# zhengjingsen/LidarDetection

Hardware: AMD Instinct MI355X
Metric: frames/sec (fwd+NMS) PointPillar-KITTI (higher is better)
Workload: dtype f32; 1 GPU; PointPillar-KITTI bs=16 per GPU, fp32, eval BN folded: HIP voxelize + PFN; dense 2D backbone = first layer from the pillars (sparse implicit GEMM), stride-1 3x3 layers as Winograd F(4x4,3x3) on the fp32 MFMA, strided deblocks as one fused MFMA GEMM (all this repo's HIP), the two stride-2 3x3 layers MIOpen, stride-1 deblock + 1x1 heads hipBLASLt; exact HIP top-k + decode + batched rotated NMS; clou; replicas=1

## Files before the change

### include/lidar_hip.h

```cpp
#ifndef LIDAR_HIP_H
#define LIDAR_HIP_H

#include <stddef.h>
#include <stdint.h>

#ifdef __cplusplus
extern "C" {
#endif

#define LIDAR_OK 0
#define LIDAR_ERR_ARG (-1)
#define LIDAR_ERR_LAUNCH (-2)
#define LIDAR_ERR_WORKSPACE (-3)
#define LIDAR_ERR_UNSUPPORTED (-4)

size_t lidar_voxelize_workspace_bytes(int batch, int n_max, int max_voxels);
int lidar_voxelize_workspace_init(void *ws, size_t ws_bytes, int batch, int n_max, int max_voxels, void *stream);
int lidar_voxelize(const float *points, const int *point_offsets, int batch, int n_max, int num_features,
                   const float *range6, const float *voxel_size3, const int *grid3, int max_points,
                   int max_voxels, int compact, int algo, float *voxels, int *coords, int *num_points,
                   int *voxel_offsets, void *ws, size_t ws_bytes, void *stream);
int lidar_voxelize_hostoff(const float *points, const int *point_offsets, const int *host_offsets, int batch, int n_max,
                           int num_features, const float *range6, const float *voxel_size3, const int *grid3, int max_points,
                           int max_voxels, int compact, int algo, float *voxels, int *coords, int *num_points,
// ... 136 lines not shown
size_t lidar_spconv_conv_table_workspace_bytes(int n, int kD, int kH, int kW, int sD, int sH, int sW);
int lidar_spconv_conv_outputs(const int *indices, int n, int batch, int D, int H, int W, int kD, int kH, int kW, int sD,
                              int sH, int sW, int pD, int pH, int pW, int *out_indices, int out_cap, int *num_out,
                              void *ws, size_t ws_bytes, void *stream);
int lidar_spconv_conv_tables(int n, int kD, int kH, int kW, int sD, int sH, int sW, int num_out, int *nbr, int *nbr_t,
                             void *ws, size_t ws_bytes, void *stream);
int lidar_spconv_grid_init(int *grid, size_t cells, void *stream);
int lidar_spconv_grid_rows(const int *indices, int n, const int *n_dev, int batch, int D, int H, int W, int *grid, int mode, void *stream);
int lidar_spconv_grid_table(const int *out_indices, int n_out, int batch, int D, int H, int W, int kD, int kH, int kW, int sD, int sH, int sW,
                            int pD, int pH, int pW, const int *grid_in, int limit, int *nbr, void *stream);
int lidar_spconv_grid_table_t(const int *indices, int n, int batch, int D, int H, int W, int kD, int kH, int kW, int sD, int sH, int sW, int pD,
                              int pH, int pW, const int *grid_out, int limit, int *nbr_t, void *stream);
int lidar_spconv_grid_pad_rows(int *out_indices, const int *num_dev, int cap, void *stream);
int lidar_spconv_transpose_table(const int *nbr, int n_out, int K, int n_in, int *nbr_t, void *stream);
size_t lidar_spconv_grid_outputs_workspace_bytes(int n, int K);
int lidar_spconv_grid_outputs(const int *indices, int n, int batch, int D, int H, int W, int kD, int kH, int kW, int sD, int sH, int sW, int pD,
                              int pH, int pW, int *grid_out, int *out_indices, int *num_out, void *ws, size_t ws_bytes,
                              void *stream);
int lidar_spconv_implicit_gemm(const float *in_features, const int *nbr, int n_out, int K, int Cin, int Cout,
                               const float *weight, const float *bias, float *out_features, void *stream);
int lidar_spconv_implicit_gemm_fused(const float *in_features, const int *nbr, int n_out, int K, int Cin, int Cout,
                                     const float *weight, const float *bias, const float *residual, int relu,
                                     float *out_features, void *stream);
int lidar_spconv_row_masks(const int *nbr, int n_out, int K, int *masks, void *stream);
size_t lidar_spconv_mask_group_workspace_bytes(int n_out);
int lidar_spconv_mask_group_init(void *ws, size_t ws_bytes, void *stream);
int lidar_spconv_mask_group(const int *nbr, int n_out, int K, int *masks, int *order, void *ws, size_t ws_bytes, void *stream);
int lidar_spconv_sorted_gemm_supported(int K, int Cin, int Cout);
int lidar_spconv_implicit_gemm_sorted(const float *in_features, const int *nbr, const int *row_mask, const int *order,
                                      int n_out, int K, int Cin, int Cout, const float *weight, const float *bias,
                                      const float *residual, int relu, float *out_features, void *stream);
size_t lidar_spconv_packed_floats(int K, int Cin, int Cout);
int lidar_spconv_pack_weights(const float *weight, int K, int Cin, int Cout, float *packed, void *stream);
int lidar_spconv_implicit_gemm_sorted_packed(const float *in_features, const int *nbr, const int *row_mask, const int *order,
                                             int n_out, int K, int Cin, int Cout, const float *packed, const float *bias,
                                             const float *residual, int relu, float *out_features, void *stream);
int lidar_spconv_wgrad(const float *in_features, const float *grad_out, const int *nbr, int n_out, int K, int Cin, int Cout,
                       float *grad_weight, void *stream);
int lidar_spconv_wgrad_mfma_supported(int K, int Cin, int Cout);
size_t lidar_spconv_wgrad_workspace_bytes(int n_out, int K, int Cin, int Cout);
int lidar_spconv_wgrad_mfma(const float *in_features, const float *grad_out, const int *nbr, const int *order, int n_out, int K,
                            int Cin, int Cout, float *grad_weight, void *ws, size_t ws_bytes, void *stream);
size_t lidar_sparse_to_dense_workspace_bytes(int batch, int D, int H, int W);
int lidar_sparse_to_dense(const float *features, const int *indices, int n, int channels, int batch, int D, int H, int W,
                          float *out, void *ws, size_t ws_bytes, void *stream);

int lidar_bias_act_nhwc(const float *in, const float *bias, long long n_pix, int C, int relu, float *out, int out_C,
                        int out_off, void *stream);
int lidar_bias_act_upsample_nhwc(const float *in, const float *bias, int batch, int h, int w, int s, int C, int relu,
                                 float *out, int out_C, int out_off, void *stream);
int lidar_dense_gemm_bias_act(const float *A, long long M, int K, const float *W, int N, const float *bias, int relu,
                              float *D, int ldd, void *ws, size_t ws_bytes, void *stream);
int lidar_dense_gemm_export_choices(int *out7, int cap);
int lidar_dense_gemm_import_choices(const int *in7, int n);

size_t lidar_wino_packed_floats(int Cin, int Cout);
int lidar_wino_supported(int Cin, int Cout);
int lidar_wino_pack_weights(const float *w, int Cin, int Cout, float *packed, void *stream);
int lidar_wino_conv3x3_nhwc(const float *in, int B, int H, int W, int Cin, const float *packed, const float *bias, int relu, int Cout,
                            float *out, int out_C, int out_off, void *stream);
int lidar_wino_conv3x3_grouped_nhwc(const float *in, int B, int H, int W, int in_C, int group_cin, int n_groups, const float *packed,
                                    const float *bias, int relu, float *out, int out_C, int out_off, void *stream);
int lidar_wino_conv3x3_grouped_compact_nhwc(const float *in, int B, int H, int W, int in_C, int group_cin, int n_groups,
                                            const float *packed, const float *bias, int relu, const int *grp_cout, const int *grp_ooff,
                                            float *out, int out_C, int out_off, void *stream);

size_t lidar_wino43_packed_floats(int Cin, int Cout);
int lidar_wino43_supported(int Cin, int Cout);
int lidar_wino43_pack_weights(const float *w, int Cin, int Cout, float *packed, void *stream);
int lidar_wino43_conv3x3_nhwc(const float *in, int B, int H, int W, int Cin, int in_C, const float *packed, const float *bias, int relu,
                              int Cout, float *out, int out_C, int out_off, void *stream);

int lidar_wino43_wgrad_supported(int Cin, int Cout);
size_t lidar_wino43_wgrad_workspace_bytes(int B, int H, int W, int Cin, int Cout);
int lidar_wino43_wgrad_nhwc(const float *x, int x_ld, const float *g, int g_ld, int B, int H, int W, int Cin, int Cout, float *dw,
                            void *ws, size_t ws_bytes, void *stream);

size_t lidar_deconv_packed_floats(int K, int N);
int lidar_deconv_supported(int K, int s, int C_up);
int lidar_deconv_pack_weights(const float *W, int K, int N, float *packed, void *stream);
int lidar_deconv_gemm_nhwc(const float *in, int B, int h, int w, int K, const float *packed, const float *bias, int relu, int s, int C_up,
                           float *out, int out_C, int out_off, void *stream);

int lidar_anchor_scores(const float *head, long long n_loc, int row_stride, int cls_off, int anchors_per_loc, int num_class,
                        float score_thresh, float *scores, unsigned char *labels, void *stream);
int lidar_decode_topk(const float *head, int batch, long long locs_per_frame, int row_stride, int box_off, int dir_off,
                      int anchors_per_loc, int num_dir_bins, const long long *top_idx, int k, const float *anchors,
                      float dir_offset, float dir_limit_offset, float period, float *boxes, void *stream);
size_t lidar_topk_workspace_bytes(int batch, long long n);
int lidar_topk_workspace_init(void *ws, size_t ws_bytes, int batch, long long n, void *stream);
int lidar_anchor_scores_hist(const float *head, int batch, long long locs_per_frame, int row_stride, int cls_off, int anchors_per_loc,
                             int num_class, float score_thresh, float *scores, unsigned char *labels, void *ws, size_t ws_bytes,
                             void *stream);
int lidar_topk_desc(const float *scores, int batch, long long n, int k, float valid_min, float score_max, int hist_ready,
                    float *top_scores, long long *top_idx, int *counts, void *ws, size_t ws_bytes, void *stream);
int lidar_post_nms_gather(const float *boxes, const float *top_scores, const long long *top_idx, const unsigned char *labels,
                          const long long *keep, const int *num_keep, int batch, int k, long long n, int keep_stride, int post,
                          float *out_boxes, float *out_scores, long long *out_labels, int *out_num, void *stream);

size_t lidar_anchor_assign_workspace_bytes(int batch, int max_gt, int num_classes);
int lidar_anchor_assign(const float *const *anchors, const long long *counts, const long long *per_loc, const long long *out_off,
                        const float *matched, const float *unmatched, const int *remap, int num_classes, int anchor_dim,
                        long long a_total, const signed char *class_of_id, const float *gt, const float *gt_enlarged, int batch,
                        int max_gt, int gt_cols, int code_size, int sincos, int norm_by_num_examples, int *labels, float *targets,
                        float *weights, void *ws, size_t ws_bytes, void *stream);

size_t lidar_anchor_loss_workspace_bytes(int batch, const long long *counts, int num_heads);
int lidar_anchor_loss_forward(const float *const *cls, const float *const *box, const float *const *dir, const long long *counts,
                              const int *cols, const int *col_off, int num_heads, const int *labels, const float *targets,
                              const float *anchors, int anchor_dim, int batch, long long n_total, int num_class, int code_size,
                              int num_dir_bins, const float *code_weights, const float *weights, int flags, float *losses, void *ws,
                              size_t ws_bytes, void *stream);
int lidar_anchor_loss_backward(const float *const *cls, const float *const *box, const float *const *dir, const long long *counts,
                               const int *cols, const int *col_off, int num_heads, const int *labels, const float *targets,
                               const float *anchors, int anchor_dim, int batch, long long n_total, int num_class, int code_size,
                               int num_dir_bins, const float *code_weights, const float *weights, int flags,
                               const float *grad_losses, float *const *d_cls, float *const *d_box, float *const *d_dir, void *ws,
                               size_t ws_bytes, void *stream);

int lidar_sparse_to_bev_nhwc(const float *features, const int *indices, int n, int channels, int batch, int D, int H, int W,
                             float *out, void *ws, size_t ws_bytes, void *stream);

int lidar_rotate_iou_eval(const float *boxes, int n, const float *query_boxes, int k, int criterion, float *iou, void *stream);

int lidar_boxes_iou_bev_cpu(const float *boxes_a, int n_a, const float *boxes_b, int n_b, float *out);
int lidar_points_in_boxes_cpu(const float *boxes, int n_boxes, const float *pts, int n_pts, int *out);

#ifdef __cplusplus
}
#endif
#endif
```

### lidardetection_amd/_lib.py

```python
import ctypes as C
import os

_HERE = os.path.dirname(os.path.abspath(__file__))
SO_PATH = os.environ.get("LIDAR_HIP_SO") or os.path.join(_HERE, "csrc", "liblidar_hip.so")

vp, i32, f32, sz = C.c_void_p, C.c_int, C.c_float, C.c_size_t

SIGNATURES = {
    "lidar_voxelize_workspace_bytes": (sz, [i32, i32, i32]),
    "lidar_voxelize_workspace_init": (i32, [vp, sz, i32, i32, i32, vp]),
    "lidar_voxelize": (i32, [vp, vp, i32, i32, i32, vp, vp, vp, i32, i32, i32, i32, vp, vp, vp, vp, vp, sz, vp]),
    "lidar_voxelize_hostoff": (i32, [vp, vp, vp, i32, i32, i32, vp, vp, vp, i32, i32, i32, i32, vp, vp, vp, vp, vp, sz, vp]),
    "lidar_voxelize_error_flag": (i32, [vp, sz, i32, i32, i32]),
    "lidar_timer_create": (vp, []),
    "lidar_timer_destroy": (None, [vp]),
    "lidar_voxelize_time_next": (None, [vp]),
    "lidar_timer_elapsed_ms": (C.c_float, [vp]),
    "lidar_timer_parts_ms": (i32, [vp, vp]),
    "lidar_voxelize_set_error_mirror": (i32, [vp, sz, i32, i32, i32, vp, vp]),
    "lidar_pillar_vfe": (i32, [vp, vp, vp, i32, vp, i32, i32, vp, vp, vp, i32, vp, vp, i32, i32, i32, vp, vp]),
    "lidar_mean_vfe": (i32, [vp, vp, i32, i32, i32, i32, vp, vp]),
    "lidar_pillar_scatter_workspace_bytes": (sz, [i32, i32, i32]),
    "lidar_pillar_scatter": (i32, [vp, vp, i32, i32, vp, i32, i32, i32, i32, i32, vp, vp, sz, vp]),
    "lidar_pillar_scatter_update": (i32, [vp, vp, i32, i32, vp, i32, i32, i32, i32, vp, vp, vp, vp]),
# ... 14 lines not shown
    "lidar_nms_batch": (i32, [vp, vp, i32, i32, f32, i32, vp, vp, vp, sz, vp]),
    "lidar_nms_batch_limited": (i32, [vp, vp, i32, i32, f32, i32, i32, vp, vp, vp, sz, vp]),
    "lidar_nms_mask_ptr": (vp, [vp, i32, i32]),
    "lidar_ball_query_stack": (i32, [i32, i32, f32, i32, vp, vp, vp, vp, vp, vp]),
    "lidar_ball_query_stack2": (i32, [i32, i32, f32, i32, f32, i32, vp, vp, vp, vp, vp, vp, vp]),
    "lidar_ball_query_grid_workspace_bytes": (sz, [i32, i32]),
    "lidar_ball_query_stack_grid": (i32, [i32, i32, i32, f32, i32, f32, i32, vp, vp, vp, vp, vp, vp, vp, sz, vp]),
    "lidar_group_points_stack": (i32, [i32, i32, i32, i32, vp, vp, vp, vp, vp, vp]),
    "lidar_group_rows_stack": (i32, [i32, i32, i32, i32, i32, i32, vp, vp, vp, vp, vp, vp, vp, vp]),
    "lidar_group_rows_affine_stack": (i32, [i32, i32, i32, i32, vp, vp, vp, vp, vp, vp, vp, vp]),
    "lidar_sa_layer2_max_supported": (i32, [i32, i32, i32]),
    "lidar_sa_layer2_max_stack": (i32, [i32, i32, i32, i32, i32, vp, vp, vp, vp, vp, vp, vp, vp, vp, vp]),
    "lidar_group_points_grad_stack": (i32, [i32, i32, i32, i32, i32, vp, vp, vp, vp, vp, vp]),
    "lidar_furthest_point_sampling": (i32, [i32, i32, i32, vp, vp, vp, vp]),
    "lidar_three_nn_stack": (i32, [i32, i32, vp, vp, vp, vp, vp, vp, vp]),
    "lidar_three_interpolate_stack": (i32, [i32, i32, vp, vp, vp, vp, vp]),
    "lidar_three_interpolate_grad_stack": (i32, [i32, i32, vp, vp, vp, vp, vp]),
    "lidar_ball_query_batch": (i32, [i32, i32, i32, f32, i32, vp, vp, vp, vp]),
    "lidar_group_points_batch": (i32, [i32, i32, i32, i32, i32, vp, vp, vp, vp]),
    "lidar_group_points_grad_batch": (i32, [i32, i32, i32, i32, i32, vp, vp, vp, vp]),
    "lidar_gather_points_batch": (i32, [i32, i32, i32, i32, vp, vp, vp, vp]),
    "lidar_gather_points_grad_batch": (i32, [i32, i32, i32, i32, vp, vp, vp, vp]),
    "lidar_three_nn_batch": (i32, [i32, i32, i32, vp, vp, vp, vp, vp]),
    "lidar_three_interpolate_batch": (i32, [i32, i32, i32, i32, vp, vp, vp, vp, vp]),
    "lidar_three_interpolate_grad_batch": (i32, [i32, i32, i32, i32, vp, vp, vp, vp, vp]),
    "lidar_roiaware_pool3d_forward": (i32, [i32, i32, i32, i32, i32, i32, i32, vp, vp, vp, vp, vp, vp, i32, vp]),
    "lidar_roiaware_pool3d_backward": (i32, [i32, i32, i32, i32, i32, i32, vp, vp, vp, vp, i32, vp]),
    "lidar_points_in_boxes": (i32, [i32, i32, i32, vp, vp, vp, vp]),
    "lidar_roipoint_pool3d_forward": (i32, [i32, i32, i32, i32, i32, vp, vp, vp, vp, vp, vp]),
    "lidar_spconv_hash_capacity": (sz, [i32]),
    "lidar_spconv_build_hash": (i32, [vp, i32, i32, i32, i32, vp, sz, vp]),
    "lidar_spconv_subm_table": (i32, [vp, i32, i32, i32, i32, i32, i32, i32, vp, sz, vp, vp]),
    "lidar_spconv_conv_table_workspace_bytes": (sz, [i32, i32, i32, i32, i32, i32, i32]),
    "lidar_spconv_conv_outputs": (i32, [vp, i32, i32, i32, i32, i32, i32, i32, i32, i32, i32, i32, i32, i32, i32, vp, i32, vp, vp, sz, vp]),
    "lidar_spconv_conv_tables": (i32, [i32, i32, i32, i32, i32, i32, i32, i32, vp, vp, vp, sz, vp]),
    "lidar_spconv_grid_init": (i32, [vp, sz, vp]),
    "lidar_spconv_grid_rows": (i32, [vp, i32, vp, i32, i32, i32, i32, vp, i32, vp]),
    "lidar_spconv_grid_table": (i32, [vp, i32, i32, i32, i32, i32, i32, i32, i32, i32, i32, i32, i32, i32, i32, vp, i32, vp, vp]),
    "lidar_spconv_grid_table_t": (i32, [vp, i32, i32, i32, i32, i32, i32, i32, i32, i32, i32, i32, i32, i32, i32, vp, i32, vp, vp]),
    "lidar_spconv_grid_pad_rows": (i32, [vp, vp, i32, vp]),
    "lidar_spconv_transpose_table": (i32, [vp, i32, i32, i32, vp, vp]),
    "lidar_spconv_grid_outputs_workspace_bytes": (sz, [i32, i32]),
    "lidar_spconv_grid_outputs": (i32, [vp, i32, i32, i32, i32, i32, i32, i32, i32, i32, i32, i32, i32, i32, i32, vp, vp, vp, vp, sz, vp]),
    "lidar_spconv_implicit_gemm": (i32, [vp, vp, i32, i32, i32, i32, vp, vp, vp, vp]),
    "lidar_spconv_implicit_gemm_fused": (i32, [vp, vp, i32, i32, i32, i32, vp, vp, vp, i32, vp, vp]),
    "lidar_spconv_row_masks": (i32, [vp, i32, i32, vp, vp]),
    "lidar_spconv_mask_group_workspace_bytes": (sz, [i32]),
    "lidar_spconv_mask_group_init": (i32, [vp, sz, vp]),
    "lidar_spconv_mask_group": (i32, [vp, i32, i32, vp, vp, vp, sz, vp]),
    "lidar_spconv_sorted_gemm_supported": (i32, [i32, i32, i32]),
    "lidar_spconv_implicit_gemm_sorted": (i32, [vp, vp, vp, vp, i32, i32, i32, i32, vp, vp, vp, i32, vp, vp]),
    "lidar_spconv_packed_floats": (sz, [i32, i32, i32]),
    "lidar_spconv_pack_weights": (i32, [vp, i32, i32, i32, vp, vp]),
    "lidar_spconv_implicit_gemm_sorted_packed": (i32, [vp, vp, vp, vp, i32, i32, i32, i32, vp, vp, vp, i32, vp, vp]),
    "lidar_spconv_wgrad": (i32, [vp, vp, vp, i32, i32, i32, i32, vp, vp]),
    "lidar_spconv_wgrad_mfma_supported": (i32, [i32, i32, i32]),
    "lidar_spconv_wgrad_workspace_bytes": (sz, [i32, i32, i32, i32]),
    "lidar_spconv_wgrad_mfma": (i32, [vp, vp, vp, vp, i32, i32, i32, i32, vp, vp, sz, vp]),
    "lidar_sparse_to_dense_workspace_bytes": (sz, [i32, i32, i32, i32]),
    "lidar_sparse_to_dense": (i32, [vp, vp, i32, i32, i32, i32, i32, i32, vp, vp, sz, vp]),
    "lidar_sparse_to_bev_nhwc": (i32, [vp, vp, i32, i32, i32, i32, i32, i32, vp, vp, sz, vp]),
    "lidar_bias_act_nhwc": (i32, [vp, vp, C.c_longlong, i32, i32, vp, i32, i32, vp]),
    "lidar_bias_act_upsample_nhwc": (i32, [vp, vp, i32, i32, i32, i32, i32, i32, vp, i32, i32, vp]),
    "lidar_dense_gemm_bias_act": (i32, [vp, C.c_longlong, i32, vp, i32, vp, i32, vp, i32, vp, sz, vp]),
    "lidar_dense_gemm_export_choices": (i32, [vp, i32]),
    "lidar_dense_gemm_import_choices": (i32, [vp, i32]),
    "lidar_wino_packed_floats": (sz, [i32, i32]),
    "lidar_wino_supported": (i32, [i32, i32]),
    "lidar_wino_pack_weights": (i32, [vp, i32, i32, vp, vp]),
    "lidar_wino_conv3x3_nhwc": (i32, [vp, i32, i32, i32, i32, vp, vp, i32, i32, vp, i32, i32, vp]),
    "lidar_wino43_packed_floats": (sz, [i32, i32]),
    "lidar_wino43_supported": (i32, [i32, i32]),
    "lidar_wino43_pack_weights": (i32, [vp, i32, i32, vp, vp]),
    "lidar_wino43_conv3x3_nhwc": (i32, [vp, i32, i32, i32, i32, i32, vp, vp, i32, i32, vp, i32, i32, vp]),
    "lidar_wino43_wgrad_supported": (i32, [i32, i32]),
    "lidar_wino43_wgrad_workspace_bytes": (sz, [i32, i32, i32, i32, i32]),
    "lidar_wino43_wgrad_nhwc": (i32, [vp, i32, vp, i32, i32, i32, i32, i32, i32, vp, vp, sz, vp]),
    "lidar_wino_conv3x3_grouped_nhwc": (i32, [vp, i32, i32, i32, i32, i32, i32, vp, vp, i32, vp, i32, i32, vp]),
    "lidar_wino_conv3x3_grouped_compact_nhwc": (i32, [vp, i32, i32, i32, i32, i32, i32, vp, vp, i32, vp, vp, vp, i32, i32, vp]),
    "lidar_deconv_packed_floats": (sz, [i32, i32]),
    "lidar_deconv_supported": (i32, [i32, i32, i32]),
    "lidar_deconv_pack_weights": (i32, [vp, i32, i32, vp, vp]),
    "lidar_deconv_gemm_nhwc": (i32, [vp, i32, i32, i32, i32, vp, vp, i32, i32, i32, vp, i32, i32, vp]),
    "lidar_anchor_scores": (i32, [vp, C.c_longlong, i32, i32, i32, i32, f32, vp, vp, vp]),
    "lidar_decode_topk": (i32, [vp, i32, C.c_longlong, i32, i32, i32, i32, i32, vp, i32, vp, f32, f32, f32, vp, vp]),
    "lidar_topk_workspace_bytes": (sz, [i32, C.c_longlong]),
    "lidar_topk_workspace_init": (i32, [vp, sz, i32, C.c_longlong, vp]),
    "lidar_anchor_scores_hist": (i32, [vp, i32, C.c_longlong, i32, i32, i32, i32, f32, vp, vp, vp, sz, vp]),
    "lidar_topk_desc": (i32, [vp, i32, C.c_longlong, i32, f32, f32, i32, vp, vp, vp, vp, sz, vp]),
    "lidar_post_nms_gather": (i32, [vp, vp, vp, vp, vp, vp, i32, i32, C.c_longlong, i32, i32, vp, vp, vp, vp, vp]),
    "lidar_anchor_assign_workspace_bytes": (sz, [i32, i32, i32]),
    "lidar_anchor_assign": (i32, [vp, vp, vp, vp, vp, vp, vp, i32, i32, C.c_longlong, vp, vp, vp, i32, i32, i32, i32, i32, i32, vp,
                                  vp, vp, vp, sz, vp]),
    "lidar_anchor_loss_workspace_bytes": (sz, [i32, vp, i32]),
    "lidar_anchor_loss_forward": (i32, [vp, vp, vp, vp, vp, vp, i32, vp, vp, vp, i32, i32, C.c_longlong, i32, i32, i32, vp, vp, i32,
                                        vp, vp, sz, vp]),
    "lidar_anchor_loss_backward": (i32, [vp, vp, vp, vp, vp, vp, i32, vp, vp, vp, i32, i32, C.c_longlong, i32, i32, i32, vp, vp, i32,
                                         vp, vp, vp, vp, vp, sz, vp]),
    "lidar_rotate_iou_eval": (i32, [vp, i32, vp, i32, i32, vp, vp]),
    "lidar_boxes_iou_bev_cpu": (i32, [vp, i32, vp, i32, vp]),
    "lidar_points_in_boxes_cpu": (i32, [vp, i32, vp, i32, vp]),
    "lidar_voxelize_cpu_scratch_bytes": (sz, [i32]),
    "lidar_voxelize_cpu": (i32, [vp, i32, i32, vp, vp, vp, i32, i32, vp, vp, vp, vp, sz]),
}

_lib = None


class LidarHipError(RuntimeError):
    pass


def lib():
    global _lib
    if _lib is None:
        if not os.path.exists(SO_PATH):
            raise LidarHipError(
                f"{SO_PATH} is missing: build it with `python -c 'import __graft_entry__ as g; g.build()'` "
                "(hipcc --offload-arch=gfx950). There is no CPU fallback.")
        _lib = C.CDLL(SO_PATH)
        for name, (res, args) in SIGNATURES.items():
            fn = getattr(_lib, name)
            fn.restype = res
            fn.argtypes = args
    return _lib


def load_variant(path):
    if not os.path.exists(path):
        raise LidarHipError(f"{path} is missing: build it with lidardetection_amd/csrc/build.py (build_variants)")
    v = C.CDLL(path)
    for name, (res, args) in SIGNATURES.items():
        fn = getattr(v, name)
        fn.restype = res
        fn.argtypes = args
    return v


def check(status, what):
    if status != 0:
        raise LidarHipError(f"{what} failed with status {status}")


def ptr(t):
    return None if t is None else C.c_void_p(t.data_ptr())


def stream():
    import torch
    try:
        return C.c_void_p(torch._C._cuda_getCurrentRawStream(torch._C._cuda_getDevice()))
    except AttributeError:
        return C.c_void_p(torch.cuda.current_stream().cuda_stream)


def host_f32(vals):
    return (C.c_float * len(vals))(*[float(v) for v in vals])


def host_i32(vals):
    return (C.c_int * len(vals))(*[int(v) for v in vals])


def require_cuda(*tensors, allow=()):
    import torch
    ok = (torch.float32, torch.int32) + tuple(allow)
# ... 15 lines not shown
```

### lidardetection_amd/bev_backbone.py

```python
import ctypes as C
import os

import torch
import torch.nn as nn
import torch.nn.functional as F

from . import _lib, wino, workspace


def bias_act_(x, bias, relu=True, out=None, out_offset=0):
    _lib.require_cuda(bias)
    if not (x.is_cuda and x.dim() == 4 and x.is_contiguous(memory_format=torch.channels_last)):
        raise _lib.LidarHipError("bias_act_: expected a channels-last CUDA tensor")
    B, C, H, W = x.shape
    if out is None:
        out, out_offset = x, 0
    elif not (out.is_contiguous(memory_format=torch.channels_last) and out.shape[0] == B and out.shape[2:] == x.shape[2:]):
        raise _lib.LidarHipError("bias_act_: output must be channels-last with the same batch / spatial shape")
    _lib.check(_lib.lib().lidar_bias_act_nhwc(_lib.ptr(x), _lib.ptr(bias), B * H * W, C, int(bool(relu)), _lib.ptr(out),
                                              out.shape[1], int(out_offset), _lib.stream()), "lidar_bias_act_nhwc")
    return out


_LT_GEMM = [os.environ.get("LIDAR_BEV_LT_GEMM", "1") != "0"]
_SPLIT_MIN = [int(os.environ.get("LIDAR_BEV_SPLIT_MIN", "8"))]
_SPLIT = [int(os.environ.get("LIDAR_BEV_SPLIT", "2"))]
_WINO = [os.environ.get("LIDAR_BEV_WINO", "1") != "0"]
_DECONV = [os.environ.get("LIDAR_BEV_DECONV", "1") != "0"]
_SPARSE_FIRST = [os.environ.get("LIDAR_BEV_SPARSE_FIRST", "1") != "0"]


def _lt_gemm(a_ptr, M, K, w_kn, bias, relu, d_ptr, ldd, device):
    ws = workspace.get("dense_gemm", 32 << 20, device)
    st = _lib.lib().lidar_dense_gemm_bias_act(a_ptr, M, K, _lib.ptr(w_kn), w_kn.shape[1], _lib.ptr(bias), int(bool(relu)), d_ptr, ldd,
                                              _lib.ptr(ws), ws.numel(), _lib.stream())
    if st == -4:
        return False
    _lib.check(st, "lidar_dense_gemm_bias_act")
    return True


def _side_streams(device, n):
    from .spconv import conv as _sc, modules as _sm
    dev = torch.device(device)
    out = []
    for pool in (_sc._SIDE_STREAMS, _sm._RULEBOOK_STREAMS)[:n]:
        st = pool.get(dev)
        if st is None:
            st = pool[dev] = torch.cuda.Stream(dev, priority=-1)
        out.append(st)
    return out


def gemm_bias_act_into_(x, w_kn, bias, out, out_offset, relu=True):
    _lib.require_cuda(w_kn, bias)
    if not (x.is_cuda and out.is_cuda and x.dtype == torch.float32 and out.dtype == torch.float32):
        raise _lib.LidarHipError("gemm_bias_act_into_: expected float32 CUDA (ROCm) tensors")
    B, K, h, w = x.shape
    N = w_kn.shape[1]
    if (not x.is_contiguous(memory_format=torch.channels_last) or not out.is_contiguous(memory_format=torch.channels_last)
            or out.shape[0] != B or out.shape[2:] != x.shape[2:] or w_kn.shape[0] != K or bias.numel() != N
            or out_offset + N > out.shape[1] or not w_kn.is_contiguous()):
        raise _lib.LidarHipError("gemm_bias_act_into_: shapes / layouts do not match")
    return _lt_gemm(_lib.ptr(x), B * h * w, K, w_kn, bias, relu, C.c_void_p(out.data_ptr() + 4 * out_offset), out.shape[1], x.device)


def rows_gemm(a2d, w_kn, bias=None, out=None):
    if _LT_GEMM[0] and a2d.is_cuda and a2d.dtype == torch.float32 and a2d.is_contiguous() and w_kn.is_contiguous():
        if out is None:
            out = torch.empty((a2d.shape[0], w_kn.shape[1]), dtype=torch.float32, device=a2d.device)
        elif not out.is_contiguous() or out.shape != (a2d.shape[0], w_kn.shape[1]):
            raise _lib.LidarHipError("rows_gemm: out must be a contiguous (M, N) tensor")
        if _lt_gemm(_lib.ptr(a2d), a2d.shape[0], a2d.shape[1], w_kn, bias, False, _lib.ptr(out), w_kn.shape[1], a2d.device):
            return out
        _LT_GEMM[0] = False
    if out is None:
        return torch.mm(a2d, w_kn) if bias is None else torch.addmm(bias, a2d, w_kn)
    return torch.mm(a2d, w_kn, out=out) if bias is None else torch.addmm(bias, a2d, w_kn, out=out)


def deconv_supported(K, s, c_up):
    return bool(_lib.lib().lidar_deconv_supported(int(K), int(s), int(c_up)))


def deconv_pack(w_kn):
    _lib.require_cuda(w_kn)
    K, N = w_kn.shape
    L = _lib.lib()
    n = L.lidar_deconv_packed_floats(K, N)
    if n == 0:
        raise _lib.LidarHipError(f"deconv_pack: unsupported shape ({K}, {N})")
    packed = torch.empty(n, dtype=torch.float32, device=w_kn.device)
    _lib.check(L.lidar_deconv_pack_weights(_lib.ptr(w_kn.contiguous()), K, N, _lib.ptr(packed), _lib.stream()), "lidar_deconv_pack_weights")
    return packed


_DECONV_MAX_BYTES = [2 ** 31 - 1]


def deconv_fits(B, K, h, w, s, out_c):
    return B * h * w * K * 4 < _DECONV_MAX_BYTES[0] and B * h * w * s * s * out_c * 4 < _DECONV_MAX_BYTES[0]


def deconv_gemm_into_(x, packed, bias, s, out, out_offset=0, relu=True):
    _lib.require_cuda(packed, bias)
    B, K, h, w = x.shape
    c_up = bias.numel()
    if not (x.is_cuda and x.dtype == torch.float32 and x.is_contiguous(memory_format=torch.channels_last) and out.is_cuda
            and out.dtype == torch.float32 and out.is_contiguous(memory_format=torch.channels_last) and out.shape[0] == B
            and tuple(out.shape[2:]) == (s * h, s * w) and 0 <= out_offset and out_offset + c_up <= out.shape[1]
            and packed.numel() == K * s * s * c_up):
        raise _lib.LidarHipError("deconv_gemm_into_: shapes / layouts do not match")
    _lib.check(_lib.lib().lidar_deconv_gemm_nhwc(_lib.ptr(x), B, h, w, K, _lib.ptr(packed), _lib.ptr(bias), int(bool(relu)), int(s), c_up,
                                                 _lib.ptr(out), out.shape[1], int(out_offset), _lib.stream()), "lidar_deconv_gemm_nhwc")
    return out


def bias_act_upsample_(y2d, bias, batch, h, w, s, out, out_offset=0, relu=True):
    _lib.require_cuda(y2d, bias)
    C = bias.numel()
    if y2d.shape != (batch * h * w, s * s * C):
        raise _lib.LidarHipError("bias_act_upsample_: GEMM output shape does not match (batch*h*w, s*s*C)")
    if not (out.is_contiguous(memory_format=torch.channels_last) and out.shape[0] == batch
            and tuple(out.shape[2:]) == (h * s, w * s)):
        raise _lib.LidarHipError("bias_act_upsample_: output must be channels-last (batch, C_out, h*s, w*s)")
    _lib.check(_lib.lib().lidar_bias_act_upsample_nhwc(_lib.ptr(y2d), _lib.ptr(bias), batch, h, w, s, C, int(bool(relu)),
                                                       _lib.ptr(out), out.shape[1], int(out_offset), _lib.stream()),
               "lidar_bias_act_upsample_nhwc")
    return out


def collect_params(*modules):
    out = []
    for m in modules:
        out += list(m.parameters()) + list(m.buffers())
    return out


def params_key(tensors):
    return tuple((t.data_ptr(), t._version) for t in tensors)


def _fold(weight, bn, out_dim, conv_bias=None):
    scale = bn.weight.detach() / torch.sqrt(bn.running_var + bn.eps)
    shift = bn.bias.detach() - bn.running_mean * scale
    if conv_bias is not None:
        shift = shift + conv_bias.detach() * scale
    shape = [1] * weight.dim()
    shape[out_dim] = -1
    return (weight.detach() * scale.view(shape)), shift.contiguous()


class _FoldedConv(tuple):

    def __new__(cls, w, b, stride, pad, packed, dilation, groups, zero_pad):
        self = super().__new__(cls, (w, b, stride, pad, packed))
        self.dilation, self.groups, self.zero_pad = dilation, groups, zero_pad
        return self


class FoldedBEVBackbone:

    def __init__(self, blocks, deblocks, heads):
        self.sources = collect_params(blocks, deblocks, *heads)
        self.source_key = params_key(self.sources)
        self.stages = []
        for blk, de in zip(blocks, deblocks):
            convs, mods, i = [], list(blk), 0
            while i < len(mods):
                zpad = (0, 0, 0, 0)
                if isinstance(mods[i], nn.ZeroPad2d):
                    zpad, i = tuple(int(v) for v in mods[i].padding), i + 1
                conv, bn = mods[i], mods[i + 1]
                assert isinstance(conv, nn.Conv2d) and isinstance(bn, nn.BatchNorm2d) and isinstance(mods[i + 2], nn.ReLU)
                assert conv.padding_mode == "zeros" and not isinstance(conv.padding, str), "FoldedBEVBackbone: explicit zero padding only"
                w, b = _fold(conv.weight, bn, 0, conv.bias)
                pad, zp = tuple(int(v) for v in conv.padding), None
                if zpad[0] == zpad[1] >= 0 and zpad[2] == zpad[3] >= 0:
                    pad = (pad[0] + zpad[2], pad[1] + zpad[0])
                else:
                    zp = zpad
                plain = tuple(conv.dilation) == (1, 1) and conv.groups == 1 and zp is None
                packed = None
                if (_WINO[0] and w.is_cuda and plain and tuple(conv.kernel_size) == (3, 3) and tuple(conv.stride) == (1, 1)
                        and pad == (1, 1) and wino.supported(w.shape[1], w.shape[0])):
                    packed = wino.pack_auto(w)
                convs.append(_FoldedConv(w.contiguous(memory_format=torch.channels_last), b, tuple(conv.stride), pad, packed,
                                         tuple(conv.dilation), conv.groups, zp))
                i += 3
            up, bn = de[0], de[1]
            assert tuple(up.dilation) == (1, 1) and up.groups == 1 and up.padding_mode == "zeros", \
                "FoldedBEVBackbone: deblocks with dilation, groups or non-zero padding modes are not supported"
            if isinstance(up, nn.ConvTranspose2d):
                w, b = _fold(up.weight, bn, 1, up.bias)
                if tuple(up.kernel_size) == tuple(up.stride) and up.stride[0] == up.stride[1] and \
                        tuple(up.padding) == (0, 0) and tuple(up.output_padding) == (0, 0):
                    w_kn = w.permute(0, 2, 3, 1).reshape(w.shape[0], -1).contiguous()
                    upc = ("gemm", w_kn, b, up.stride[0])
                    if (_DECONV[0] and w.is_cuda and up.stride[0] > 1 and deconv_supported(w_kn.shape[0], up.stride[0], b.numel())):
                        upc = ("deconv_mfma", (deconv_pack(w_kn), w_kn), b, up.stride[0])
                else:
                    upc = ("deconv", w.contiguous(memory_format=torch.channels_last), b, (up.stride, up.padding, up.output_padding))
            else:
                w, b = _fold(up.weight, bn, 0, up.bias)
                upc = ("conv", w.contiguous(memory_format=torch.channels_last), b, (up.stride, up.padding))
            self.stages.append((convs, upc))
        self.up_channels = [s[1][2].numel() for s in self.stages]
        for h in heads:
            assert tuple(h.kernel_size) == (1, 1) and tuple(h.stride) == (1, 1)
        self.head_split = [h.weight.shape[0] for h in heads]
        if heads:
            self.head_wt = torch.cat([h.weight.detach().flatten(1) for h in heads], 0).t().contiguous()
            self.head_b = torch.cat([h.bias.detach() if h.bias is not None else h.weight.new_zeros(h.weight.shape[0])
                                     for h in heads], 0).contiguous()
        self._cats = {}
        self._streams = None
        self._first_sparse = None
        c0 = self.stages[0][0][0]
        w0, b0, st0, pad0, _ = c0
        k0 = w0.shape[2]
        if (w0.is_cuda and w0.shape[2] == w0.shape[3] and st0[0] == st0[1] and pad0[0] == pad0[1] and k0 * k0 <= 31
                and c0.dilation == (1, 1) and c0.groups == 1 and c0.zero_pad is None):
            from .spconv import ops as _sops
            if _sops.sorted_gemm_supported(k0 * k0, w0.shape[1], w0.shape[0]):
                self._first_sparse = (w0.permute(2, 3, 1, 0).reshape(k0 * k0, w0.shape[1], w0.shape[0]).contiguous(), b0, k0, int(st0[0]), int(pad0[0]))

    def first_layer_from_pillars(self, pm):
        from . import pillar_ops
        from .spconv import ops as _sops
        w9, b0, k0, st0, pad0 = self._first_sparse
        nbr, OH, OW = pillar_ops.pillar_conv_table(pm.coords, pm.B, pm.nx, pm.ny, k0, st0, pad0, pm.num_voxels_dev)
        order = _sops.mask_order(nbr)
        out = _sops.indice_conv_fused(pm.features, nbr, w9, b0, None, True, order)
        return out.view(pm.B, OH, OW, w9.shape[2]).permute(0, 3, 1, 2)

    def sparse_first_ok(self):
        return self._first_sparse is not None and _SPARSE_FIRST[0]

    def features(self, canvas, slot=0, first_done=False):
        x, cat, off = canvas, None, 0
        for si, (convs, (kind, uw, ub, ustride)) in enumerate(self.stages):
            for ci, cv in enumerate(convs):
                if first_done and si == 0 and ci == 0:
                    continue
                w, b, stride, pad, packed = cv
                if packed is not None and _WINO[0] and x.is_contiguous(memory_format=torch.channels_last):
                    x = wino.conv3x3_auto(x, packed, w.shape[0], b, True)
                    continue
                if cv.zero_pad is not None:
                    x = F.pad(x, cv.zero_pad)
                x = F.conv2d(x, w, None, stride, pad, cv.dilation, cv.groups)
                if not x.is_contiguous(memory_format=torch.channels_last):
                    x = x.contiguous(memory_format=torch.channels_last)
                bias_act_(x, b)
            B, _, h, w = x.shape
            y = None
            if kind == "deconv_mfma":
                oh, ow = h * ustride, w * ustride
                if not deconv_fits(B, x.shape[1], h, w, ustride, sum(self.up_channels)):
                    kind, uw = "gemm", uw[1]
                    y = rows_gemm(x.permute(0, 2, 3, 1).reshape(B * h * w, -1), uw)
                else:
                    uw = uw[0]
            elif kind == "gemm":
                oh, ow = h * ustride, w * ustride
                if not (ustride == 1 and _LT_GEMM[0]):
                    y = rows_gemm(x.permute(0, 2, 3, 1).reshape(B * h * w, -1), uw)
            else:
                y = F.conv_transpose2d(x, uw, None, *ustride) if kind == "deconv" else F.conv2d(x, uw, None, *ustride)
                if not y.is_contiguous(memory_format=torch.channels_last):
                    y = y.contiguous(memory_format=torch.channels_last)
                oh, ow = y.shape[2], y.shape[3]
            if cat is None:
                shape = (B, sum(self.up_channels), oh, ow)
                cat = self._cats.get(slot)
                if cat is None or cat.shape != shape or cat.device != x.device:
                    cat = self._cats[slot] = torch.empty(shape, dtype=torch.float32, device=x.device,
                                                         memory_format=torch.channels_last)
            if kind == "gemm" and y is None:
                if not gemm_bias_act_into_(x, uw, ub, cat, off):
                    _LT_GEMM[0] = False
                    y = rows_gemm(x.permute(0, 2, 3, 1).reshape(B * h * w, -1), uw)
            if kind == "deconv_mfma":
                deconv_gemm_into_(x, uw, ub, ustride, cat, off)
            elif kind == "gemm":
                if y is not None:
                    bias_act_upsample_(y, ub, B, h, w, ustride, cat, off)
            else:
                bias_act_(y, ub, out=cat, out_offset=off)
            off += ub.numel()
        return cat

    def stale(self):
        return params_key(self.sources) != self.source_key

    def merged(self, canvas):
        first_done = False
        if not torch.is_tensor(canvas):
            if self.sparse_first_ok():
                canvas, first_done = self.first_layer_from_pillars(canvas), True
            else:
                canvas = canvas.dense()
        B = canvas.shape[0]
        if 1 < _SPLIT[0] <= 2 and canvas.is_cuda and B % _SPLIT[0] == 0 and B // _SPLIT[0] >= _SPLIT_MIN[0]:
            return self._merged_split(canvas, _SPLIT[0], first_done)
        cat = self.features(canvas, first_done=first_done)
        B, C, H, W = cat.shape
        out = rows_gemm(cat.permute(0, 2, 3, 1).reshape(B * H * W, C), self.head_wt, self.head_b)
        return out.view(B, H, W, -1)

    def _merged_split(self, canvas, n, first_done=False):
        dev = canvas.device
        cur = torch.cuda.current_stream(dev)
        self._streams = _side_streams(dev, n)
        B, hb = canvas.shape[0], canvas.shape[0] // n
        out = None
        for i, st in enumerate(self._streams):
            st.wait_stream(cur)
            with torch.cuda.stream(st):
                cat = self.features(canvas[i * hb:(i + 1) * hb], slot=i + 1, first_done=first_done)
                _, C, H, W = cat.shape
                if out is None:
                    with torch.cuda.stream(cur):
                        out = torch.empty((B, H, W, self.head_wt.shape[1]), dtype=torch.float32, device=dev)
                    st.wait_stream(cur)
                out.record_stream(st)
                rows_gemm(cat.permute(0, 2, 3, 1).reshape(hb * H * W, C), self.head_wt, self.head_b, out=out[i * hb:(i + 1) * hb].view(hb * H * W, -1))
        for st in self._streams:
            cur.wait_stream(st)
        return out

    def __call__(self, canvas):
        return torch.split(self.merged(canvas), self.head_split, dim=-1)
```

Before: 3224 frames/s.

## Add custom fp32 MFMA GEMM kernel for the 1x1 detection heads

Replaces the hipBLASLt/torch GEMM for the merged 1x1 head convolutions with a dedicated HIP kernel. Packed weights stay resident in LDS, A rows are streamed through buffer loads with a three-stage register prefetch across persistent tiles, and the kernel is XCD-aware. Bias is fused into an LDS-staged coalesced store. It targets the skinny-N head GEMM that library kernels handle poorly, at the cost of a large hand-scheduled kernel limited to K≤384, N≤80.

```diff
diff --git a/include/lidar_hip.h b/include/lidar_hip.h
--- a/include/lidar_hip.h
+++ b/include/lidar_hip.h
@@ -242,6 +242,12 @@
 int lidar_deconv_gemm_nhwc(const float *in, int B, int h, int w, int K, const float *packed, const float *bias, int relu, int s, int C_up,
                            float *out, int out_C, int out_off, void *stream);
 
+int lidar_head_gemm_supported(int K, int N);
+size_t lidar_head_gemm_packed_floats(int K, int N);
+int lidar_head_gemm_pack_weights(const float *w_kn, int K, int N, float *packed, void *stream);
+int lidar_head_gemm_rows(const float *a, long long M, int K, int lda, const float *packed, const float *bias, int N, float *d, int ldd,
+                         void *stream);
+
 int lidar_anchor_scores(const float *head, long long n_loc, int row_stride, int cls_off, int anchors_per_loc, int num_class,
                         float score_thresh, float *scores, unsigned char *labels, void *stream);
 int lidar_decode_topk(const float *head, int batch, long long locs_per_frame, int row_stride, int box_off, int dir_off,
diff --git a/lidardetection_amd/_lib.py b/lidardetection_amd/_lib.py
--- a/lidardetection_amd/_lib.py
+++ b/lidardetection_amd/_lib.py
@@ -120,6 +120,10 @@
     "lidar_deconv_supported": (i32, [i32, i32, i32]),
     "lidar_deconv_pack_weights": (i32, [vp, i32, i32, vp, vp]),
     "lidar_deconv_gemm_nhwc": (i32, [vp, i32, i32, i32, i32, vp, vp, i32, i32, i32, vp, i32, i32, vp]),
+    "lidar_head_gemm_supported": (i32, [i32, i32]),
+    "lidar_head_gemm_packed_floats": (sz, [i32, i32]),
+    "lidar_head_gemm_pack_weights": (i32, [vp, i32, i32, vp, vp]),
+    "lidar_head_gemm_rows": (i32, [vp, C.c_longlong, i32, i32, vp, vp, i32, vp, i32, vp]),
     "lidar_anchor_scores": (i32, [vp, C.c_longlong, i32, i32, i32, i32, f32, vp, vp, vp]),
     "lidar_decode_topk": (i32, [vp, i32, C.c_longlong, i32, i32, i32, i32, i32, vp, i32, vp, f32, f32, f32, vp, vp]),
     "lidar_topk_workspace_bytes": (sz, [i32, C.c_longlong]),
diff --git a/lidardetection_amd/bev_backbone.py b/lidardetection_amd/bev_backbone.py
--- a/lidardetection_amd/bev_backbone.py
+++ b/lidardetection_amd/bev_backbone.py
@@ -28,6 +28,7 @@
 _WINO = [os.environ.get("LIDAR_BEV_WINO", "1") != "0"]
 _DECONV = [os.environ.get("LIDAR_BEV_DECONV", "1") != "0"]
 _SPARSE_FIRST = [os.environ.get("LIDAR_BEV_SPARSE_FIRST", "1") != "0"]
+_HEAD_GEMM = [os.environ.get("LIDAR_BEV_HEAD_GEMM", "1") != "0"]
 
 
 def _lt_gemm(a_ptr, M, K, w_kn, bias, relu, d_ptr, ldd, device):
@@ -77,6 +78,44 @@
     if out is None:
         return torch.mm(a2d, w_kn) if bias is None else torch.addmm(bias, a2d, w_kn)
     return torch.mm(a2d, w_kn, out=out) if bias is None else torch.addmm(bias, a2d, w_kn, out=out)
+
+
+def head_gemm_supported(K, N):
+    return bool(_lib.lib().lidar_head_gemm_supported(int(K), int(N)))
+
+
+def head_gemm_pack(w_kn):
+    _lib.require_cuda(w_kn)
+    K, N = w_kn.shape
+    L = _lib.lib()
+    n = L.lidar_head_gemm_packed_floats(K, N)
+    if n == 0:
+        raise _lib.LidarHipError(f"head_gemm_pack: unsupported shape ({K}, {N})")
+    packed = torch.empty(n, dtype=torch.float32, device=w_kn.device)
+    _lib.check(L.lidar_head_gemm_pack_weights(_lib.ptr(w_kn), K, N, _lib.ptr(packed), _lib.stream()), "lidar_head_gemm_pack_weights")
+    return packed
+
+
+_HEAD_GEMM_MAX_BYTES = [2 ** 31 - 1]
+HEAD_GEMM_CALLS = [0]
+
+
+def head_gemm_fits(M, lda, ldd):
+    return M * lda * 4 < _HEAD_GEMM_MAX_BYTES[0] and M * ldd * 4 < _HEAD_GEMM_MAX_BYTES[0]
+
+
+def head_gemm_rows(a2d, packed, bias, N, out=None):
+    _lib.require_cuda(packed, bias)
+    M, K = a2d.shape
+    if out is None:
+        out = torch.empty((M, N), dtype=torch.float32, device=a2d.device)
+    if not (a2d.is_cuda and a2d.dtype == torch.float32 and a2d.stride(1) == 1 and out.is_cuda and out.dtype == torch.float32
+            and out.shape == (M, N) and out.stride(1) == 1 and (bias is None or bias.numel() == N)):
+        raise _lib.LidarHipError("head_gemm_rows: shapes / layouts do not match")
+    _lib.check(_lib.lib().lidar_head_gemm_rows(_lib.ptr(a2d), M, K, a2d.stride(0), _lib.ptr(packed), _lib.ptr(bias), N, _lib.ptr(out),
+                                               out.stride(0), _lib.stream()), "lidar_head_gemm_rows")
+    HEAD_GEMM_CALLS[0] += 1
+    return out
 
 
 def deconv_supported(K, s, c_up):
@@ -213,6 +252,9 @@
             self.head_wt = torch.cat([h.weight.detach().flatten(1) for h in heads], 0).t().contiguous()
             self.head_b = torch.cat([h.bias.detach() if h.bias is not None else h.weight.new_zeros(h.weight.shape[0])
                                      for h in heads], 0).contiguous()
+            self.head_packed = None
+            if _HEAD_GEMM[0] and self.head_wt.is_cuda and head_gemm_supported(*self.head_wt.shape):
+                self.head_packed = head_gemm_pack(self.head_wt)
         self._cats = {}
         self._streams = None
         self._first_sparse = None
@@ -294,6 +336,12 @@
     def stale(self):
         return params_key(self.sources) != self.source_key
 
+    def _heads(self, a2d, out=None):
+        N = self.head_wt.shape[1]
+        if _HEAD_GEMM[0] and self.head_packed is not None and head_gemm_fits(a2d.shape[0], a2d.stride(0), N if out is None else out.stride(0)):
+            return head_gemm_rows(a2d, self.head_packed, self.head_b, N, out)
+        return rows_gemm(a2d, self.head_wt, self.head_b, out=out)
+
     def merged(self, canvas):
         first_done = False
         if not torch.is_tensor(canvas):
@@ -306,7 +354,7 @@
             return self._merged_split(canvas, _SPLIT[0], first_done)
         cat = self.features(canvas, first_done=first_done)
         B, C, H, W = cat.shape
-        out = rows_gemm(cat.permute(0, 2, 3, 1).reshape(B * H * W, C), self.head_wt, self.head_b)
+        out = self._heads(cat.permute(0, 2, 3, 1).reshape(B * H * W, C))
         return out.view(B, H, W, -1)
 
     def _merged_split(self, canvas, n, first_done=False):
@@ -325,7 +373,7 @@
                         out = torch.empty((B, H, W, self.head_wt.shape[1]), dtype=torch.float32, device=dev)
                     st.wait_stream(cur)
                 out.record_stream(st)
-                rows_gemm(cat.permute(0, 2, 3, 1).reshape(hb * H * W, C), self.head_wt, self.head_b, out=out[i * hb:(i + 1) * hb].view(hb * H * W, -1))
+                self._heads(cat.permute(0, 2, 3, 1).reshape(hb * H * W, C), out=out[i * hb:(i + 1) * hb].view(hb * H * W, -1))
         for st in self._streams:
             cur.wait_stream(st)
         return out
diff --git a/lidardetection_amd/csrc/head_gemm.hip b/lidardetection_amd/csrc/head_gemm.hip
--- /dev/null
+++ b/lidardetection_amd/csrc/head_gemm.hip
@@ -0,0 +1,216 @@
+#include "common.h"
+
+typedef float f32x4 __attribute__((ext_vector_type(4)));
+typedef unsigned u32x4 __attribute__((ext_vector_type(4)));
+
+#define HG_OOB 0x80000000u
+#define HG_MT 8
+#define HG_ROWS (16 * HG_MT)
+
+static inline int hg_nt(int N) { return (N + 15) >> 4; }
+
+static inline int hg_nc3(int K) { return ((K >> 4) + 2) / 3 * 3; }
+
+__global__ __launch_bounds__(256) void hg_pack_kernel(const float *__restrict__ W, int K, int N, int NT, int n_floats, float *__restrict__ P) {
+    const int idx = (int)(blockIdx.x * 256 + threadIdx.x);
+    if (idx >= n_floats) return;
+    const int j = idx & 3, lane = (idx >> 2) & 63, ct = idx >> 8, t = ct % NT, c = ct / NT;
+    const int k = 16 * c + 4 * (lane >> 4) + j, col = 16 * t + (lane & 15);
+    P[idx] = (col < N && k < K) ? W[(size_t)k * N + col] : 0.f;
+}
+
+struct HgArgs {
+    const float *a;
+    const float *pk;
+    const float *bias;
+    float *d;
+    int M, K, N, lda, ldd;
+    int n_tiles;
+    unsigned a_bytes, d_bytes;
+};
+
+template <int NT> static constexpr int hg_stg_pitch() { return 16 * NT + 4; }
+static size_t hg_lds_bytes(int K, int NT) { return (size_t)hg_nc3(K) * NT * 1024 + (size_t)4 * 16 * (16 * NT + 4) * 4; }
+
+template <int NT>
+__global__ __launch_bounds__(256) void hg_gemm_kernel(const HgArgs a) {
+    extern __shared__ float4 s_mem4[];
+    const int t = threadIdx.x, l = t & 63, wv = __builtin_amdgcn_readfirstlane(t >> 6);
+    const int NC = a.K >> 4;
+    constexpr int PITCH = hg_stg_pitch<NT>();
+    const int n_b4 = (NC + 2) / 3 * 3 * NT * 64;
+    const f32x4 *s_b = reinterpret_cast<const f32x4 *>(s_mem4);
+    float *stg = reinterpret_cast<float *>(s_mem4 + n_b4) + wv * 16 * PITCH;
+
+    const int nt8 = (a.n_tiles + 7) >> 3;
+    const int xcd = (int)(blockIdx.x & 7), slot = (int)(blockIdx.x >> 3), stride = (int)(gridDim.x >> 3) * 4;
+    const int tile_end = min((xcd + 1) * nt8, a.n_tiles);
+    if (xcd * nt8 + slot * 4 >= tile_end) return;
+    for (int i = t; i < n_b4; i += 256) s_mem4[i] = reinterpret_cast<const float4 *>(a.pk)[i];
+    __syncthreads();
+    int tile = xcd * nt8 + slot * 4 + wv;
+    if (tile >= tile_end) return;
+
+    const __amdgpu_buffer_rsrc_t arsrc = __builtin_amdgcn_make_buffer_rsrc(const_cast<float *>(a.a), (short)0, (int)a.a_bytes, 0x00020000);
+    const __amdgpu_buffer_rsrc_t drsrc = __builtin_amdgcn_make_buffer_rsrc(a.d, (short)0, (int)a.d_bytes, 0x00020000);
+
+    float bv[NT];
+#pragma unroll
+    for (int n = 0; n < NT; ++n) bv[n] = (a.bias && 16 * n + (l & 15) < a.N) ? a.bias[16 * n + (l & 15)] : 0.f;
+    const int N4 = a.N >> 2;
+    int e_row[NT];
+    unsigned e_lds[NT], e_off[NT];
+#pragma unroll
+    for (int e = 0; e < NT; ++e) {
+        const int i = l + 64 * e, r = i / N4, q = i - r * N4;
+        e_row[e] = i < 16 * N4 ? r : 0x40000000;
+        e_lds[e] = (unsigned)((r & 15) * PITCH + 4 * q);
+        e_off[e] = (unsigned)r * (unsigned)a.ldd * 4u + 16u * (unsigned)q;
+    }
+
+    const int NC3 = (NC + 2) / 3 * 3;
+    unsigned voff[HG_MT], nvoff[HG_MT];
+    auto set_voff = [&](unsigned (&vo)[HG_MT], int tl) {
+#pragma unroll
+        for (int m = 0; m < HG_MT; ++m) {
+            const int row = tl * HG_ROWS + 16 * m + (l & 15);
+            vo[m] = (tl < tile_end && row < a.M) ? (unsigned)row * (unsigned)a.lda * 4u + 16u * (unsigned)(l >> 4) : HG_OOB;
+        }
+    };
+    auto issue = [&](f32x4 (&dst)[HG_MT], const unsigned (&vo)[HG_MT], int c) {
+        const bool real = c < NC;
+#pragma unroll
+        for (int m = 0; m < HG_MT; ++m)
+            dst[m] = __builtin_bit_cast(f32x4, __builtin_amdgcn_raw_buffer_load_b128(arsrc, (int)(real ? vo[m] : HG_OOB), real ? c * 64 : 0, 0));
+    };
+
+    f32x4 a0[HG_MT], a1[HG_MT], a2[HG_MT], bq[NT];
+    set_voff(voff, tile);
+    issue(a0, voff, 0);
+    issue(a1, voff, 1);
+#pragma unroll
+    for (int n = 0; n < NT; ++n) bq[n] = s_b[n * 64 + l];
+
+    for (;;) {
+        const int tile_next = tile + stride;
+        set_voff(nvoff, tile_next);
+        f32x4 acc[HG_MT][NT];
+#pragma unroll
+        for (int m = 0; m < HG_MT; ++m)
+#pragma unroll
+            for (int n = 0; n < NT; ++n) acc[m][n] = f32x4{0.f, 0.f, 0.f, 0.f};
+        asm volatile("s_nop 7" ::: "memory");
+#define HG_CHUNK(c, AC, AFILL, VO, CF)                                                                                             \
+    {                                                                                                                              \
+        issue(AFILL, VO, CF);                                                                                                      \
+        const int cn_ = (c) + 1 == NC3 ? 0 : (c) + 1;                                                                              \
+        __builtin_amdgcn_sched_barrier(0);                                                                                         \
+        _Pragma("unroll") for (int n = 0; n < NT; ++n) {                                                                           \
+            _Pragma("unroll") for (int j = 0; j < 4; ++j)                                                                          \
+                _Pragma("unroll") for (int m = 0; m < HG_MT; ++m)                                                                  \
+                    asm volatile("v_mfma_f32_16x16x4_f32 %0, %1, %2, %0" : "+a"(acc[m][n]) : "v"(AC[m][j]), "v"(bq[n][j]));       \
+            bq[n] = s_b[(cn_ * NT + n) * 64 + l];                                                                                  \
+            __builtin_amdgcn_sched_barrier(0);                                                                                     \
+        }                                                                                                                          \
+    }
+        int c = 0;
+        for (; c < NC3 - 3; c += 3) {
+            HG_CHUNK(c, a0, a2, voff, c + 2)
+            HG_CHUNK(c + 1, a1, a0, voff, c + 3)
+            HG_CHUNK(c + 2, a2, a1, voff, c + 4)
+        }
+        HG_CHUNK(c, a0, a2, voff, c + 2)
+        HG_CHUNK(c + 1, a1, a0, nvoff, 0)
+        HG_CHUNK(c + 2, a2, a1, nvoff, 1)
+#undef HG_CHUNK
+        const int row0 = tile * HG_ROWS;
+        asm volatile("s_nop 15\n\ts_nop 15" ::: "memory");
+#pragma unroll
+        for (int m = 0; m < HG_MT; ++m) {
+#pragma unroll
+            for (int n = 0; n < NT; ++n)
+#pragma unroll
+                for (int r = 0; r < 4; ++r) stg[(4 * (l >> 4) + r) * PITCH + 16 * n + (l & 15)] = acc[m][n][r] + bv[n];
+            asm volatile("" ::: "memory");
+            __builtin_amdgcn_sched_barrier(0);
+            const int lim = a.M - row0 - 16 * m;
+            const int soff = (row0 + 16 * m) * a.ldd * 4;
+            f32x4 sv[NT];
+#pragma unroll
+            for (int e = 0; e < NT; ++e) sv[e] = *reinterpret_cast<const f32x4 *>(stg + e_lds[e]);
+#pragma unroll
+            for (int e = 0; e < NT; ++e)
+                __builtin_amdgcn_raw_buffer_store_b128(__builtin_bit_cast(u32x4, sv[e]), drsrc, (int)(e_row[e] < lim ? e_off[e] : HG_OOB), lim > 0 ? soff : 0, 0);
+            asm volatile("" ::: "memory");
+            __builtin_amdgcn_sched_barrier(0);
+        }
+        if (tile_next >= tile_end) break;
+        tile = tile_next;
+        for (int m = 0; m < HG_MT; ++m) voff[m] = nvoff[m];
+    }
+}
+
+LIDAR_EXPORT int lidar_head_gemm_supported(int K, int N) { return K >= 16 && K <= 384 && (K & 15) == 0 && N >= 4 && N <= 80 && (N & 3) == 0; }
+
+LIDAR_EXPORT size_t lidar_head_gemm_packed_floats(int K, int N) {
+    if (!lidar_head_gemm_supported(K, N)) return 0;
+    return (size_t)hg_nc3(K) * hg_nt(N) * 256;
+}
+
+LIDAR_EXPORT int lidar_head_gemm_pack_weights(const float *w_kn, int K, int N, float *packed, void *stream) {
+    if (!lidar_head_gemm_supported(K, N)) return LIDAR_ERR_UNSUPPORTED;
+    if (!w_kn || !packed || (reinterpret_cast<uintptr_t>(packed) & 15)) return LIDAR_ERR_ARG;
+    const int NT = hg_nt(N);
+    const int n_floats = hg_nc3(K) * NT * 256;
+    hipLaunchKernelGGL(hg_pack_kernel, dim3(divup(n_floats, 256)), dim3(256), 0, (hipStream_t)stream, w_kn, K, N, NT, n_floats, packed);
+    return lidar_check_launch("lidar_head_gemm_pack_weights");
+}
+
+static int hg_cu_count() {
+    static int cus[64] = {};
+    int dev = 0, n = 0;
+    if (hipGetDevice(&dev) != hipSuccess) return 256;
+    dev &= 63;
+    if (cus[dev] == 0) cus[dev] = (hipDeviceGetAttribute(&n, hipDeviceAttributeMultiprocessorCount, dev) == hipSuccess && n > 0) ? n : 256;
+    return cus[dev];
+}
+
+template <int NT>
+static int hg_launch(const HgArgs &a, unsigned grid, hipStream_t stream) {
+    static bool attr_set[64] = {};
+    int dev_id = 0;
+    (void)hipGetDevice(&dev_id);
+    dev_id &= 63;
+    if (!attr_set[dev_id]) {
+        (void)hipFuncSetAttribute(reinterpret_cast<const void *>(&hg_gemm_kernel<NT>), hipFuncAttributeMaxDynamicSharedMemorySize, (int)hg_lds_bytes(384, NT));
+        attr_set[dev_id] = true;
+    }
+    hipLaunchKernelGGL(hg_gemm_kernel<NT>, dim3(grid), dim3(256), hg_lds_bytes(a.K, NT), stream, a);
+    return lidar_check_launch("lidar_head_gemm_rows");
+}
+
+LIDAR_EXPORT int lidar_head_gemm_rows(const float *a, long long M, int K, int lda, const float *packed, const float *bias, int N, float *d,
+                                      int ldd, void *stream) {
+    if (!lidar_head_gemm_supported(K, N)) return LIDAR_ERR_UNSUPPORTED;
+    if (!a || !packed || !d || M <= 0 || lda < K || ldd < N || (lda & 3) || (ldd & 3)) return LIDAR_ERR_ARG;
+    if ((reinterpret_cast<uintptr_t>(a) & 15) || (reinterpret_cast<uintptr_t>(packed) & 15) || (reinterpret_cast<uintptr_t>(d) & 15) ||
+        (reinterpret_cast<uintptr_t>(bias) & 15))
+        return LIDAR_ERR_ARG;
+    if (M * lda * 4 >= 0x7fffffffll || M * ldd * 4 >= 0x7fffffffll) return LIDAR_ERR_UNSUPPORTED;
+    HgArgs g;
+    g.a = a; g.pk = packed; g.bias = bias; g.d = d;
+    g.M = (int)M; g.K = K; g.N = N; g.lda = lda; g.ldd = ldd;
+    g.n_tiles = divup(M, HG_ROWS);
+    g.a_bytes = (unsigned)((M - 1) * lda * 4 + (long long)K * 4);
+    g.d_bytes = (unsigned)((M - 1) * ldd * 4 + (long long)N * 4);
+    long long want = (((long long)divup(g.n_tiles, 4) + 7) / 8) * 8;
+    const long long cap = ((long long)hg_cu_count() / 8) * 8;
+    if (cap >= 8 && want > cap) want = cap;
+    switch (hg_nt(N)) {
+    case 1: return hg_launch<1>(g, (unsigned)want, (hipStream_t)stream);
+    case 2: return hg_launch<2>(g, (unsigned)want, (hipStream_t)stream);
+    case 3: return hg_launch<3>(g, (unsigned)want, (hipStream_t)stream);
+    case 4: return hg_launch<4>(g, (unsigned)want, (hipStream_t)stream);
+    default: return hg_launch<5>(g, (unsigned)want, (hipStream_t)stream);
+    }
+}
```

Measured after the change: 3252 frames/s (median of 6 runs). Within noise of the previous version (+0.9%).
